# baggepinnen/LPVSpectral.jl

Measured on AMD Instinct MI355X. Metric: signals/sec, ls_sparse_spectral_lpv group lasso N=2^20 Nf=512 Nv=8 (2000 ADMM iters; iters/sec in admm_iters_per_sec), higher is better.
Workload: dtype f64

## Files before the change

lpvspectral.jl_amd/csrc/api.hip:

```cpp
#include <cmath>
#include <cstdarg>
#include <cstdio>
#include <cstdlib>
#include <cstring>
#include <ctime>
#include <map>
#include <mutex>
#include <array>
#include <thread>
#include <string>
#include <vector>

#include "lpvs_internal.h"

namespace lpvs {

static thread_local char g_err[512] = "";

void set_error(const char *fmt, ...) {
    va_list ap;
    va_start(ap, fmt);
    vsnprintf(g_err, sizeof(g_err), fmt, ap);
    va_end(ap);
}
// ... 582 lines not shown
    if (lpvs_device_count() == 0) { set_error("no HIP device visible (the gfx950 path has no CPU fallback)"); return LPVS_EDEVICE; }
    hipStream_t s = nullptr;
    const int64_t nreg = z ? 2 * Nf - 1 : 2 * Nf;
    DevArg dt, df; DevOut dA;
    LPVS_TRY(dt.set(t, N, s)); LPVS_TRY(df.set(f, Nf, s)); LPVS_TRY(dA.set(A_out, N * nreg));
    LPVS_TRY(launch_fourier_regressor_colmajor(dt.p, N, df.p, Nf, (int)z, dA.p, s));
    return dA.finish(s);
}

int32_t lpvs_basis_activation_f64(const double *V, int64_t N, int64_t Nv, int32_t normalize, int32_t coulomb, double *K_out) {
    if (lpvs_device_count() == 0) { set_error("no HIP device visible (the gfx950 path has no CPU fallback)"); return LPVS_EDEVICE; }
    if (N <= 0 || Nv <= 0) { set_error("N and Nv must be positive"); return LPVS_EARGUMENT; }
    hipStream_t s = nullptr;
    const int64_t nb = coulomb ? 2 * Nv : Nv;
    DevArg dV; LPVS_TRY(dV.set(V, N, s));
    double lo, hi, am, gamma; std::vector<double> vc;
    LPVS_TRY(device_minmax(dV.p, N, &lo, &hi, &am, s));
    basis_centers(lo, hi, am, Nv, coulomb, vc, &gamma);
    DevBuf dvc, Kt; LPVS_TRY(dvc.alloc(sizeof(double) * vc.size()));
    LPVS_TRY(copy_to_device(dvc.p, vc.data(), sizeof(double) * vc.size(), s));
    LPVS_TRY(Kt.alloc(sizeof(double) * (size_t)N * (size_t)nb));
    LPVS_TRY(launch_basis_table(dV.p, N, dvc.as<double>(), nb, gamma, normalize, coulomb, Kt.as<double>(), nb, s));
    std::vector<double> hk((size_t)N * nb), ho((size_t)N * nb);
    LPVS_TRY(copy_from_device(hk.data(), Kt.p, sizeof(double) * hk.size(), s));
    for (int64_t n = 0; n < N; ++n) for (int64_t j = 0; j < nb; ++j) ho[n + j * N] = hk[n * nb + j];
    if (is_device_ptr(K_out)) { LPVS_HIP(hipMemcpy(K_out, ho.data(), sizeof(double) * ho.size(), hipMemcpyHostToDevice)); }
    else memcpy(K_out, ho.data(), sizeof(double) * ho.size());
    return LPVS_OK;
}

static int32_t build_lpv_tables(const double *dX, const double *dV, int64_t N, int64_t Npad, const double *dw, int64_t Nf,
                                int64_t Nv, int normalize, int coulomb, DevBuf &T, DevBuf &K, int64_t *ldk_out, hipStream_t s,
                                const double *ranges = nullptr) {
    const int64_t nb = coulomb ? 2 * Nv : Nv, ldk = nb + 1;
    double lo, hi, am, gamma; std::vector<double> vc;
    if (ranges) { lo = ranges[0]; hi = ranges[1]; am = ranges[2]; }
    else LPVS_TRY(device_minmax(dV, N, &lo, &hi, &am, s));
    basis_centers(lo, hi, am, Nv, coulomb, vc, &gamma);
    DevBuf dvc; LPVS_TRY(dvc.alloc(sizeof(double) * vc.size()));
    LPVS_TRY(copy_to_device(dvc.p, vc.data(), sizeof(double) * vc.size(), s));
    LPVS_TRY(T.alloc(sizeof(double2) * (size_t)Npad * (size_t)Nf));
    LPVS_TRY(K.alloc(sizeof(double) * (size_t)Npad * (size_t)ldk));
    if (Npad > N) {
        LPVS_HIP(hipMemsetAsync(T.as<double2>() + N * Nf, 0, sizeof(double2) * (size_t)(Npad - N) * (size_t)Nf, s));
        LPVS_HIP(hipMemsetAsync(K.as<double>() + N * ldk, 0, sizeof(double) * (size_t)(Npad - N) * (size_t)ldk, s));
    }
    LPVS_TRY(launch_trig_table(dX, N, dw, Nf, T.as<double2>(), s));
    LPVS_TRY(launch_basis_table(dV, N, dvc.as<double>(), nb, gamma, normalize, coulomb, K.as<double>(), ldk, s));
    LPVS_HIP(hipStreamSynchronize(s));
    *ldk_out = ldk;
    return LPVS_OK;
}

int32_t lpvs_lpv_regressor_f64(const double *X, const double *V, int64_t N, const double *w, int64_t Nf, int64_t Nv,
                               int32_t normalize, int32_t coulomb, int32_t permuted, double *Phi_out) {
    if (lpvs_device_count() == 0) { set_error("no HIP device visible (the gfx950 path has no CPU fallback)"); return LPVS_EDEVICE; }
    if (N <= 0 || Nf <= 0 || Nv <= 0) { set_error("N, Nf and Nv must be positive"); return LPVS_EARGUMENT; }
    hipStream_t s = nullptr;
    const int64_t nb = coulomb ? 2 * Nv : Nv;
    DevArg dX, dV, dw; DevOut dP;
    LPVS_TRY(dX.set(X, N, s)); LPVS_TRY(dV.set(V, N, s)); LPVS_TRY(dw.set(w, Nf, s));
    LPVS_TRY(dP.set(Phi_out, N * 2 * Nf * nb));
    DevBuf T, K; int64_t ldk;
    LPVS_TRY(build_lpv_tables(dX.p, dV.p, N, N, dw.p, Nf, Nv, normalize, coulomb, T, K, &ldk, s));
    LPVS_TRY(launch_lpv_regressor_colmajor(T.as<double2>(), K.as<double>(), ldk, N, Nf, nb, permuted, dP.p, s));
    return dP.finish(s);
}

struct ApSlots {
    bool ok = false;
    double emax = 0;
    int64_t nf8 = 0, s8 = 0, nsl = 0;
    bool merged = false;
    int64_t s0 = 0;
    double delta = 0;
    std::vector<double> eps, om_hi, om_lo, omr_hi, omr_lo;
    ApStep step{};
};
static thread_local bool g_f32_admission = false;

static ApSlots make_ap_slots(const std::vector<double> &hw, double xam) {
    ApSlots sl;
    const int64_t Nf = (int64_t)hw.size();
    const long double a0 = hw[0], D = Nf > 1 ? ((long double)hw[Nf - 1] - (long double)hw[0]) / (long double)(Nf - 1) : 0.0L;
    sl.eps.resize((size_t)Nf);
    for (int64_t f = 0; f < Nf; ++f) {
        sl.eps[f] = (double)((long double)hw[f] - (a0 + (long double)f * D));
        sl.emax = std::fmax(sl.emax, std::fabs(sl.eps[f]));
    }
    double wam = 0;
    for (double v : hw) wam = std::fmax(wam, std::fabs(v));
    sl.ok = std::isfinite(sl.emax) && std::isfinite(xam) && sl.emax * xam <= 1e-7;
    if (!sl.ok && g_f32_admission && std::isfinite(sl.emax) && std::isfinite(xam) && sl.emax <= 0x1p-23 * wam) {
        sl.ok = true;
        if (sl.emax * xam > 3e-3) for (auto &e : sl.eps) e = 0.0;
    }
    if (!sl.ok) return sl;
    sl.nf8 = round_up(Nf, 8); sl.s8 = round_up(2 * Nf - 1, 8); sl.nsl = sl.nf8 + sl.s8;
    auto split = [](long double v, double &hi, double &lo) { hi = (double)v; lo = (double)(v - (long double)hi); };
    sl.omr_hi.resize((size_t)sl.nf8); sl.omr_lo.resize((size_t)sl.nf8);
    sl.s0 = sl.nf8;
    bool merged = false;
    if (Nf > 1 && D != 0.0L) {
        const long double j0r = 2.0L * a0 / D;
        const long long j0 = llroundl(j0r);
        const long double delta = 2.0L * a0 - (long double)j0 * D;
        if (j0 >= 0 && j0 < Nf && std::fabs((double)delta) * xam <= 1e-7) {
            merged = true; sl.merged = true;
            sl.s0 = j0; sl.delta = (double)delta;
            sl.nsl = round_up(j0 + 2 * Nf - 1, 8);
            sl.s8 = sl.nsl;
        }
    }
    sl.om_hi.resize((size_t)sl.nsl); sl.om_lo.resize((size_t)sl.nsl);
    if (merged) {
        for (int64_t j = 0; j < sl.nsl; ++j) split((long double)j * D, sl.om_hi[j], sl.om_lo[j]);
    } else {
        for (int64_t m = 0; m < sl.nf8; ++m) split((long double)m * D, sl.om_hi[m], sl.om_lo[m]);
        for (int64_t q = 0; q < sl.s8; ++q) split(2.0L * a0 + (long double)q * D, sl.om_hi[sl.nf8 + q], sl.om_lo[sl.nf8 + q]);
    }
    for (int64_t f = 0; f < sl.nf8; ++f) split(a0 + (long double)f * D, sl.omr_hi[f], sl.omr_lo[f]);
    for (int b = 0; b < 8; ++b) split((long double)b * D, sl.step.hi[b], sl.step.lo[b]);
    return sl;
}
struct ApSlotsDev {
    DevBuf hi, lo, rhi, rlo, eps;
    int32_t upload(const ApSlots &sl, hipStream_t s) {
        LPVS_TRY(hi.alloc(sizeof(double) * (size_t)sl.nsl)); LPVS_TRY(lo.alloc(sizeof(double) * (size_t)sl.nsl));
        LPVS_TRY(rhi.alloc(sizeof(double) * (size_t)sl.nf8)); LPVS_TRY(rlo.alloc(sizeof(double) * (size_t)sl.nf8));
        LPVS_TRY(eps.alloc(sizeof(double) * sl.eps.size()));
        LPVS_TRY(copy_to_device(hi.p, sl.om_hi.data(), sizeof(double) * (size_t)sl.nsl, s));
        LPVS_TRY(copy_to_device(lo.p, sl.om_lo.data(), sizeof(double) * (size_t)sl.nsl, s));
        LPVS_TRY(copy_to_device(rhi.p, sl.omr_hi.data(), sizeof(double) * (size_t)sl.nf8, s));
        LPVS_TRY(copy_to_device(rlo.p, sl.omr_lo.data(), sizeof(double) * (size_t)sl.nf8, s));
        LPVS_TRY(copy_to_device(eps.p, sl.eps.data(), sizeof(double) * sl.eps.size(), s));
        return LPVS_OK;
    }
};

static int32_t create_lpv_impl(const double *y, int64_t ns, const double *X, const double *V, int64_t N, const double *w, int64_t Nf,
                               int64_t Nv, int32_t normalize, int32_t coulomb, int32_t device, lpvs_problem **out,
                               const double *ranges = nullptr) {
    if (N <= 0 || Nf <= 0 || Nv <= 0 || ns <= 0) { set_error("N, Nf, Nv and the number of signals must be positive"); return LPVS_EARGUMENT; }
    lpvs_problem *h = nullptr;
    LPVS_TRY(problem_begin(device, out, &h));
    struct Guard { lpvs_problem *h; ~Guard() { delete h; } } guard{h};
    hipStream_t s = h->stream;
    const int64_t nb = coulomb ? 2 * Nv : Nv;
    h->kind = 1; h->N = N; h->Nf = Nf; h->nb = nb; h->n = 2 * Nf * nb; h->np = round_up(h->n, 128); h->ns = ns;
    DevArg dy, dX, dV, dw;
    LPVS_TRY(dy.set(y, N * ns, s)); LPVS_TRY(dX.set(X, N, s)); LPVS_TRY(dV.set(V, N, s)); LPVS_TRY(dw.set(w, Nf, s));
    LPVS_TRY(h->G.alloc(sizeof(double) * (size_t)h->np * (size_t)h->np));
    LPVS_TRY(h->b.alloc(sizeof(double) * (size_t)h->np * (size_t)ns));
    LPVS_HIP(hipMemsetAsync(h->G.p, 0, h->G.bytes, s));
    LPVS_HIP(hipMemsetAsync(h->b.p, 0, h->b.bytes, s));
    LPVS_TRY(alloc_state(h));

    const int form_opt = option_in_effect(LPVS_OPT_GRAM_FORM, h->opt[LPVS_OPT_GRAM_FORM]);
    const std::string form = form_opt == LPVS_GRAM_AP ? "ap" : form_opt == LPVS_GRAM_KRS ? "krs" : form_opt == LPVS_GRAM_KR ? "kr" : "auto";
    bool use_ap = false;
    ApSlots sl;
    double xam = 0;
    if (form == "auto" || form == "ap") {
        std::vector<double> hw;
        LPVS_TRY(fetch_host(hw, w, Nf));
        double xlo, xhi;
        if (ranges) xam = ranges[3];
        else LPVS_TRY(device_minmax(dX.p, N, &xlo, &xhi, &xam, s));
        sl = make_ap_slots(hw, xam);
        use_ap = sl.ok;
        if (form == "ap" && !use_ap) { set_error("LPVS_GRAM_FORM=ap but w is not an arithmetic progression (max|eps|*max|x| = %.3g)", sl.emax * xam); return LPVS_EARGUMENT; }
    }
    if (use_ap) {
        const int64_t nf8 = sl.nf8, nsl = sl.nsl, P = nb * (nb + 1) / 2;
        const ApStep &step = sl.step;
        double lo, hi, am, gamma; std::vector<double> vc;
        DevBuf K, KK, dvc, part, tab, tabb, nwork, epsr;
        ApSlotsDev sd;
        DrainOnExit drain(s);
        LPVS_HIP(hipEventRecord(h->ev[0].a, s));
        if (ranges) { lo = ranges[0]; hi = ranges[1]; am = ranges[2]; }
        else LPVS_TRY(device_minmax(dV.p, N, &lo, &hi, &am, s));
        basis_centers(lo, hi, am, Nv, coulomb, vc, &gamma);
        const int64_t ldk = nb + 1;
        LPVS_TRY(dvc.alloc(sizeof(double) * vc.size()));
        LPVS_TRY(copy_to_device(dvc.p, vc.data(), sizeof(double) * vc.size(), s));
        LPVS_TRY(K.alloc(sizeof(double) * (size_t)N * (size_t)ldk));
        LPVS_TRY(KK.alloc(sizeof(double) * (size_t)N * (size_t)P));
        LPVS_TRY(launch_basis_table(dV.p, N, dvc.as<double>(), nb, gamma, normalize, coulomb, K.as<double>(), ldk, s));
        LPVS_TRY(launch_pair_table(K.as<double>(), ldk, nb, N, KK.as<double>(), s));
        LPVS_TRY(sd.upload(sl, s));
        LPVS_HIP(hipEventRecord(h->ev[0].b, s));
        LPVS_TRY(part.alloc(std::max(nudft_partial_bytes(N, nsl, P), nudft_partial_bytes(N, nf8, nb))));
        LPVS_TRY(tab.alloc(sizeof(double) * (size_t)nsl * (size_t)P * 4));
        LPVS_TRY(tabb.alloc(sizeof(double) * (size_t)nf8 * (size_t)nb * 4));
        LPVS_HIP(hipEventRecord(h->ev[1].a, s));
        const bool nufft_on = option_in_effect(LPVS_OPT_SLOT_SUMS, h->opt[LPVS_OPT_SLOT_SUMS]) != LPVS_SLOTS_DIRECT;
        bool nufft = nufft_on && sl.merged && nufft_applicable(N, nsl, P);
        const int nfg = nufft_grid_size(nsl);
        const double xam_ = xam;
        if (nufft) {
            LPVS_TRY(nwork.alloc(nufft_work_bytes(N, nsl, P)));
            const int32_t rc = launch_nufft_tab(dX.p, nullptr, N, xam_, KK.as<double>(), P, (int)P, step.hi[1], step.lo[1], 0, (int)nsl, nfg, false, nwork.p,
                                                tab.as<double>(), s);
            if (rc == kNufftNonFinite) nufft = false;
            else if (rc != LPVS_OK) return rc;
        }
        if (nufft) {
            h->gram_form = 5;
        } else {
            h->gram_form = 4;
            LPVS_TRY(launch_nudft(dX.p, nullptr, N, KK.as<double>(), P, (int)P, sd.hi.as<double>(), sd.lo.as<double>(), (int)nsl, step, part.as<double>(), tab.as<double>(), s));
        }
        LPVS_TRY(launch_ap_assemble(tab.as<double>(), sd.eps.as<double>(), Nf, sl.s0, sl.delta, nb, h->n, h->G.as<double>(), h->np, s));
        LPVS_HIP(hipEventRecord(h->ev[1].b, s));
        LPVS_HIP(hipEventRecord(h->ev[2].a, s));
        const bool nufft_rhs = nufft && sl.s0 % 2 == 0 && (int)(sl.s0 / 2 + nf8) <= (int)nsl;
        if (nufft_rhs) {
            std::vector<double> er(sl.eps.size());
            for (size_t f = 0; f < er.size(); ++f) er[f] = sl.eps[f] + 0.5 * sl.delta;
            LPVS_TRY(epsr.alloc(sizeof(double) * er.size()));
            LPVS_TRY(copy_to_device(epsr.p, er.data(), sizeof(double) * er.size(), s));
            LPVS_HIP(hipStreamSynchronize(s));
        }
        for (int64_t q = 0; q < ns; ++q) {
            bool by_nufft = nufft_rhs;
            if (by_nufft) {
                const int32_t rc = launch_nufft_tab(dX.p, dy.p + q * N, N, xam_, K.as<double>(), ldk, (int)nb, step.hi[1], step.lo[1], (int)(sl.s0 / 2), (int)nf8, nfg,
                                                    true, nwork.p, tabb.as<double>(), s);
                if (rc == kNufftNonFinite) by_nufft = false;
                else if (rc != LPVS_OK) return rc;
            }
            if (!by_nufft)
                LPVS_TRY(launch_nudft(dX.p, dy.p + q * N, N, K.as<double>(), ldk, (int)nb, sd.rhi.as<double>(), sd.rlo.as<double>(), (int)nf8, step, part.as<double>(), tabb.as<double>(), s));
            LPVS_TRY(launch_ap_rhs(tabb.as<double>(), by_nufft ? epsr.as<double>() : sd.eps.as<double>(), Nf, nb, h->b.as<double>() + q * h->np, s));
        }
        LPVS_HIP(hipEventRecord(h->ev[2].b, s));
        LPVS_HIP(hipStreamSynchronize(s));
        h->t_basis = h->ev[0].ms(); h->t_gram = h->ev[1].ms(); h->t_reduce = h->ev[2].ms();
        h->gram_launches = 8.0 * (double)N * (double)nsl * (double)P;
        h->gram_flops = (double)N * (double)h->n * (double)(h->n + 1);
        guard.h = nullptr;
        *out = h;
        return LPVS_OK;
    }

    const bool krs = form != "kr" && gram_krs_fits(nb);
    const GramPlan pl = krs ? make_gram_plan_pairs(Nf, nb, N) : make_gram_plan(h->n, N);
    const int64_t Npad = pl.ksplit * pl.rows_per_chunk;

    DevBuf T, K, KK, G3, slab, scr; int64_t ldk;
    DrainOnExit drain(s);
    LPVS_HIP(hipEventRecord(h->ev[0].a, s));
    LPVS_TRY(build_lpv_tables(dX.p, dV.p, N, Npad, dw.p, Nf, Nv, normalize, coulomb, T, K, &ldk, s, ranges));
    if (krs) {
        LPVS_TRY(KK.alloc(sizeof(double) * (size_t)Npad * (size_t)pl.pairs));
        LPVS_TRY(launch_pair_table(K.as<double>(), ldk, nb, Npad, KK.as<double>(), s));
    }
    LPVS_HIP(hipEventRecord(h->ev[0].b, s));
    LPVS_TRY(slab.alloc(pl.slab_bytes));
    LPVS_TRY(scr.alloc(rhs_scratch_bytes(N, h->n)));
    if (krs) LPVS_TRY(G3.alloc(sizeof(double) * (size_t)pl.np2 * (size_t)(pl.np2 * pl.pairs)));
    struct Side { hipStream_t s = nullptr; hipEvent_t ready = nullptr, done = nullptr;
                  ~Side() { if (s) { (void)hipStreamSynchronize(s); (void)hipStreamDestroy(s); } if (ready) (void)hipEventDestroy(ready); if (done) (void)hipEventDestroy(done); } } side;
    LPVS_HIP(hipStreamCreateWithFlags(&side.s, hipStreamNonBlocking));
    LPVS_HIP(hipEventCreateWithFlags(&side.ready, hipEventDisableTiming));
    LPVS_HIP(hipEventCreateWithFlags(&side.done, hipEventDisableTiming));
    LPVS_HIP(hipEventRecord(side.ready, s));
    LPVS_HIP(hipStreamWaitEvent(side.s, side.ready, 0));
    LPVS_HIP(hipEventRecord(h->ev[1].a, s));
    if (krs) LPVS_TRY(launch_gram_krs(pl, T.as<double2>(), Nf, KK.as<double>(), nb, slab.as<double>(), s));
    else LPVS_TRY(launch_gram_kr(pl, T.as<double2>(), Nf, K.as<double>(), ldk, nb, slab.as<double>(), s));
    LPVS_HIP(hipEventRecord(h->ev[1].b, s));
    for (int64_t q = 0; q < ns; ++q)
        LPVS_TRY(launch_rhs_kr(T.as<double2>(), Nf, K.as<double>(), ldk, nb, dy.p + q * N, N, h->b.as<double>() + q * h->np, scr.as<double>(), scr.bytes, side.s));
    LPVS_HIP(hipEventRecord(side.done, side.s));
    LPVS_HIP(hipEventRecord(h->ev[2].a, s));
    if (krs) LPVS_TRY(launch_gram_reduce_krs(pl, slab.as<double>(), nb, G3.as<double>(), h->G.as<double>(), h->np, s));
    else LPVS_TRY(launch_gram_reduce(pl, slab.as<double>(), h->G.as<double>(), h->np, s));
    LPVS_HIP(hipStreamWaitEvent(s, side.done, 0));
    LPVS_HIP(hipEventRecord(h->ev[2].b, s));
    LPVS_HIP(hipStreamSynchronize(s));
    h->t_basis = h->ev[0].ms(); h->t_gram = h->ev[1].ms(); h->t_reduce = h->ev[2].ms();
    h->gram_launches = (double)pl.tiles * 128.0 * 256.0 * 2.0 * (double)(pl.ksplit * pl.rows_per_chunk); h->gram_flops = (double)N * (double)h->n * (double)(h->n + 1);
    h->gram_form = krs ? 2 : 1;
    guard.h = nullptr;
    *out = h;
    return LPVS_OK;
}

int32_t lpvs_problem_create_lpv_f64(const double *y, const double *X, const double *V, int64_t N, const double *w, int64_t Nf,
                                    int64_t Nv, int32_t normalize, int32_t coulomb, int32_t device, lpvs_problem **out) {
    return create_lpv_impl(y, 1, X, V, N, w, Nf, Nv, normalize, coulomb, device, out);
}

int32_t lpvs_problem_create_lpv_multi_f64(const double *Y, int64_t ns, const double *X, const double *V, int64_t N, const double *w,
                                          int64_t Nf, int64_t Nv, int32_t normalize, int32_t coulomb, int32_t device,
                                          lpvs_problem **out) {
    return create_lpv_impl(Y, ns, X, V, N, w, Nf, Nv, normalize, coulomb, device, out);
}

int32_t lpvs_lpv_ranges_f64(const double *X, const double *V, int64_t N, double *out4) {
    if (!X || !V || !out4 || N <= 0) { set_error("NULL argument or N <= 0"); return LPVS_EARGUMENT; }
    if (lpvs_device_count() == 0) { set_error("no HIP device visible (the gfx950 path has no CPU fallback)"); return LPVS_EDEVICE; }
    hipStream_t s = nullptr;
    DevArg dX, dV;
    LPVS_TRY(dX.set(X, N, s)); LPVS_TRY(dV.set(V, N, s));
    double xlo, xhi;
    LPVS_TRY(device_minmax(dV.p, N, &out4[0], &out4[1], &out4[2], s));
    LPVS_TRY(device_minmax(dX.p, N, &xlo, &xhi, &out4[3], s));
    return LPVS_OK;
}

int32_t lpvs_problem_create_lpv_rows_f64(const double *Y, int64_t ns, const double *X, const double *V, int64_t N_local, const double *w,
                                         int64_t Nf, int64_t Nv, int32_t normalize, int32_t coulomb, const double *ranges4,
                                         int32_t device, lpvs_problem **out) {
    if (!ranges4) { set_error("ranges4 is NULL"); return LPVS_EARGUMENT; }
    if (!(ranges4[0] <= ranges4[1]) || !(ranges4[2] >= 0) || !(ranges4[3] >= 0)) { set_error("ranges4 = {min V, max V, max|V|, max|X|} is inconsistent"); return LPVS_EARGUMENT; }
    return create_lpv_impl(Y, ns, X, V, N_local, w, Nf, Nv, normalize, coulomb, device, out, ranges4);
}

int32_t lpvs_problem_device_gram_f64(lpvs_problem *h, double **G_dev, double **b_dev, int64_t *np) {
    if (!h) { set_error("NULL handle"); return LPVS_EARGUMENT; }
    if (G_dev) *G_dev = h->G.as<double>();
    if (b_dev) *b_dev = h->b.as<double>();
    if (np) *np = h->np;
    return LPVS_OK;
}

int32_t lpvs_problem_gram_modified(lpvs_problem *h) {
    if (!h) { set_error("NULL handle"); return LPVS_EARGUMENT; }
    h->M_valid = false; h->Mp_valid = false; h->inited = false;
    h->drop_graph();
    return LPVS_OK;
}

int32_t lpvs_problem_create_fourier_f64(const double *y, const double *t, int64_t N, const double *f, int64_t Nf, const double *W,
                                        int32_t device, lpvs_problem **out) {
    if (N <= 0 || Nf <= 0) { set_error("N and Nf must be positive"); return LPVS_EARGUMENT; }
    int64_t zf = 0;
    LPVS_TRY(lpvs_check_freq_f64(f, Nf, &zf));
    lpvs_problem *h = nullptr;
    LPVS_TRY(problem_begin(device, out, &h));
    struct Guard { lpvs_problem *h; ~Guard() { delete h; } } guard{h};
    hipStream_t s = h->stream;
    h->kind = 0; h->N = N; h->Nf = Nf; h->zerofreq = zf; h->n = zf ? 2 * Nf - 1 : 2 * Nf;
    DevArg dt, df;
    LPVS_TRY(dt.set(t, N, s)); LPVS_TRY(df.set(f, Nf, s));
    const int form_opt = option_in_effect(LPVS_OPT_GRAM_FORM, h->opt[LPVS_OPT_GRAM_FORM]);
    const std::string form = form_opt == LPVS_GRAM_AP ? "ap" : form_opt == LPVS_GRAM_KRS ? "krs" : form_opt == LPVS_GRAM_KR ? "kr" : "auto";
    if (form == "auto" || form == "ap") {
        std::vector<double> hw;
        LPVS_TRY(fetch_host(hw, f, Nf));
        for (auto &v : hw) v = 6.283185307179586 * v;
        double tlo, thi, tam;
        LPVS_TRY(device_minmax(dt.p, N, &tlo, &thi, &tam, s));
        const ApSlots sl = make_ap_slots(hw, tam);
        if (form == "ap" && !sl.ok) { set_error("LPVS_GRAM_FORM=ap but 2*pi*f is not an arithmetic progression (max|eps|*max|t| = %.3g)", sl.emax * tam); return LPVS_EARGUMENT; }
        if (sl.ok) {
            h->np = round_up(h->n, 128);
            DevArg dy, dW;
            LPVS_TRY(dy.set(y, N, s));
            if (W) LPVS_TRY(dW.set(W, N, s));
            LPVS_TRY(h->G.alloc(sizeof(double) * (size_t)h->np * (size_t)h->np));
            LPVS_TRY(h->b.alloc(sizeof(double) * (size_t)h->np));
            LPVS_HIP(hipMemsetAsync(h->G.p, 0, h->G.bytes, s));
            LPVS_HIP(hipMemsetAsync(h->b.p, 0, h->b.bytes, s));
            LPVS_TRY(alloc_state(h));
            ApSlotsDev sd; DevBuf part, tab, tabb;
            DrainOnExit drain(s);
            LPVS_HIP(hipEventRecord(h->ev[0].a, s));
            LPVS_TRY(sd.upload(sl, s));
            LPVS_HIP(hipEventRecord(h->ev[0].b, s));
            LPVS_TRY(part.alloc(std::max(nudft_partial_bytes(N, sl.nsl, 1), nudft_partial_bytes(N, sl.nf8, 1))));
            LPVS_TRY(tab.alloc(sizeof(double) * (size_t)sl.nsl * 4));
            LPVS_TRY(tabb.alloc(sizeof(double) * (size_t)sl.nf8 * 4));
            const double *Wd = W ? dW.p : nullptr;
            LPVS_HIP(hipEventRecord(h->ev[1].a, s));
            LPVS_TRY(launch_nudft(dt.p, nullptr, N, Wd, 1, 1, sd.hi.as<double>(), sd.lo.as<double>(), (int)sl.nsl, sl.step, part.as<double>(), tab.as<double>(), s));
            LPVS_TRY(launch_ap_assemble_fourier(tab.as<double>(), sd.eps.as<double>(), Nf, sl.s0, sl.delta, (int)zf, h->n, h->G.as<double>(), h->np, 1, 0, 0, s));
            LPVS_HIP(hipEventRecord(h->ev[1].b, s));
            LPVS_HIP(hipEventRecord(h->ev[2].a, s));
            LPVS_TRY(launch_nudft(dt.p, dy.p, N, Wd, 1, 1, sd.rhi.as<double>(), sd.rlo.as<double>(), (int)sl.nf8, sl.step, part.as<double>(), tabb.as<double>(), s));
            LPVS_TRY(launch_ap_rhs_fourier(tabb.as<double>(), sd.eps.as<double>(), Nf, (int)zf, h->b.as<double>(), 1, 0, 0, s));
            LPVS_HIP(hipEventRecord(h->ev[2].b, s));
            LPVS_HIP(hipStreamSynchronize(s));
            h->t_basis = h->ev[0].ms(); h->t_gram = h->ev[1].ms(); h->t_reduce = h->ev[2].ms();
            h->gram_launches = 8.0 * (double)N * (double)sl.nsl;
            h->gram_flops = (double)N * (double)h->n * (double)(h->n + 1);
            h->gram_form = 4;
            guard.h = nullptr;
            *out = h;
            return LPVS_OK;
        }
    }
    LPVS_TRY(create_panel_problem(h, y, W, N, [&](double *P, int64_t ld) {
        return launch_fourier_panel(dt.p, N, df.p, Nf, (int)zf, P, ld, s);
    }));
    guard.h = nullptr;
// ... 1444 lines not shown
```

lpvspectral.jl_amd/csrc/nudft.hip:

```cpp
#include "lpvs_internal.h"

#include <cstdlib>

namespace lpvs {

namespace {

constexpr int RB = 16;

template <int QPT, int S>
__global__ void __launch_bounds__(256)
nudft_accumulate_kernel(const double *__restrict__ x, const double *__restrict__ y, int64_t N, const double *__restrict__ Wt,
                        int64_t ldw, int nq, const double *__restrict__ om_hi, const double *__restrict__ om_lo, int nslots,
                        const ApStep step, double *__restrict__ out, const int64_t *__restrict__ seg, int64_t rows_per_chunk) {
    constexpr int SLOTS = 64 * S, NA = 8 * S;
    constexpr int WSTR = (QPT + 1) & ~1;
    constexpr int NEF = NA + 8;
    __shared__ __attribute__((aligned(16))) double wrow[2][RB][4 * WSTR];
    __shared__ __attribute__((aligned(16))) double ef[2][RB][NEF][2];
    __shared__ double xs[2][RB], ys[2][RB];
    const int t = threadIdx.x;
    const int sl = t & 63;
    const int g = __builtin_amdgcn_readfirstlane(t >> 6);
    const int slot0 = blockIdx.x * SLOTS;
// ... 41 lines not shown
            }
            ef[buf][pr][pk][0] = c; ef[buf][pr][pk][1] = sn;
        }
        for (int e = t; e < RB * 4 * QPT; e += 256) {
            const int pr = e / (4 * QPT), q = e - pr * (4 * QPT);
            const int64_t r = rb + pr;
            const double wv = (r < r1 && q < nqb) ? (Wt ? Wt[(r - wbase) * ldw + qbase + q] : 1.0) : 0.0;
            wrow[buf][pr][(q / QPT) * WSTR + q % QPT] = wv;
        }
        __syncthreads();
        if (nvalid > 0) {
#pragma unroll
            for (int rr = 0; rr < RB; ++rr) {
                const double yv = ys[buf][rr], xv = xs[buf][rr];
                double tv[S][4];
#pragma unroll
                for (int u = 0; u < S; ++u) {
                    const int ls = sl + 64 * u;
                    const double2 e2 = *reinterpret_cast<const double2 *>(&ef[buf][rr][ls >> 3][0]);
                    const double2 f2 = *reinterpret_cast<const double2 *>(&ef[buf][rr][NA + (ls & 7)][0]);
                    const double c = fma(e2.x, f2.x, -(e2.y * f2.y)) * yv, sn = fma(e2.y, f2.x, e2.x * f2.y) * yv;
                    tv[u][0] = c; tv[u][1] = sn; tv[u][2] = xv * c; tv[u][3] = xv * sn;
                }
                double wq[WSTR];
#pragma unroll
                for (int q = 0; q < WSTR; q += 2) {
                    const double2 w2 = *reinterpret_cast<const double2 *>(&wrow[buf][rr][g * WSTR + q]);
                    wq[q] = w2.x; wq[q + 1] = w2.y;
                }
#pragma unroll
                for (int q = 0; q < QPT; ++q)
#pragma unroll
                    for (int u = 0; u < S; ++u) {
                        acc[u][q][0] = fma(wq[q], tv[u][0], acc[u][q][0]);
                        acc[u][q][1] = fma(wq[q], tv[u][1], acc[u][q][1]);
                        acc[u][q][2] = fma(wq[q], tv[u][2], acc[u][q][2]);
                        acc[u][q][3] = fma(wq[q], tv[u][3], acc[u][q][3]);
                    }
            }
        }
    }
    if (nvalid > 0) {
#pragma unroll
        for (int u = 0; u < S; ++u) {
            const int slot = slot0 + sl + 64 * u;
            if (slot >= nslots) continue;
            double *o = out + (((int64_t)blockIdx.y * nslots + slot) * nq + qbase + q0) * 4;
#pragma unroll
            for (int q = 0; q < QPT; ++q)
                if (q < nvalid) {
#pragma unroll
                    for (int v = 0; v < 4; ++v) o[q * 4 + v] = acc[u][q][v];
                }
        }
    }
}


template <int S>
__global__ void __launch_bounds__(256)
nudft_single_kernel(const double *__restrict__ x, const double *__restrict__ y, int64_t N, const double *__restrict__ Wt, int64_t ldw,
                    const double *__restrict__ om_hi, const double *__restrict__ om_lo, int nslots, const ApStep step,
                    double *__restrict__ out, const int64_t *__restrict__ seg, int64_t rows_per_chunk) {
    constexpr int NA = 8 * S, NEF = NA + 8;
    __shared__ __attribute__((aligned(16))) double ef[2][RB][NEF][2];
    __shared__ double xs[2][RB], ws[2][RB];
    __shared__ __attribute__((aligned(16))) double comb[3][64 * S][4];
    const int t = threadIdx.x, sl = t & 63;
    const int g = __builtin_amdgcn_readfirstlane(t >> 6);
    const int slot0 = blockIdx.x * 64 * S;
    int64_t r0 = (int64_t)blockIdx.y * rows_per_chunk;
    int64_t r1 = r0 + rows_per_chunk < N ? r0 + rows_per_chunk : N;
    int64_t wbase = 0;
    if (seg != nullptr) { r0 = seg[3 * blockIdx.y]; r1 = seg[3 * blockIdx.y + 1]; wbase = seg[3 * blockIdx.y + 2]; }
    double acc[S][4];
#pragma unroll
    for (int u = 0; u < S; ++u)
#pragma unroll
        for (int v = 0; v < 4; ++v) acc[u][v] = 0.0;
    int buf = 0;
    for (int64_t rb = r0; rb < r1; rb += RB, buf ^= 1) {
        for (int e = t; e < RB * NEF; e += 256) {
            const int pr = e / NEF, pk = e - pr * NEF;
            double wh, wl;
            if (pk < NA) {
                const int as = slot0 + 8 * pk;
                const bool ok = as < nslots;
                wh = ok ? om_hi[as] : 0.0; wl = ok ? om_lo[as] : 0.0;
            } else {
                wh = step.hi[pk - NA]; wl = step.lo[pk - NA];
            }
            const int64_t r = rb + pr;
            double c = 1.0, sn = 0.0;
            if (r < r1) {
                const double xv = x[r];
                const double p = wh * xv;
                const double d = fma(wh, xv, -p) + wl * xv;
                sincos(p, &sn, &c);
                const double c2 = fma(-d, sn, c), s2 = fma(d, c, sn);
                c = c2; sn = s2;
                if (pk == 0) { xs[buf][pr] = xv; ws[buf][pr] = (Wt ? Wt[(r - wbase) * ldw] : 1.0) * (y ? y[r] : 1.0); }
            } else if (pk == 0) {
                xs[buf][pr] = 0.0; ws[buf][pr] = 0.0;
            }
            ef[buf][pr][pk][0] = c; ef[buf][pr][pk][1] = sn;
        }
        __syncthreads();
#pragma unroll
        for (int i = 0; i < RB / 4; ++i) {
            const int rr = g + 4 * i;
            const double wv = ws[buf][rr], xv = xs[buf][rr];
#pragma unroll
            for (int u = 0; u < S; ++u) {
                const int ls = sl + 64 * u;
                const double2 e2 = *reinterpret_cast<const double2 *>(&ef[buf][rr][ls >> 3][0]);
                const double2 f2 = *reinterpret_cast<const double2 *>(&ef[buf][rr][NA + (ls & 7)][0]);
                const double c = fma(e2.x, f2.x, -(e2.y * f2.y)) * wv, sn = fma(e2.y, f2.x, e2.x * f2.y) * wv;
                acc[u][0] += c; acc[u][1] += sn;
                acc[u][2] = fma(xv, c, acc[u][2]); acc[u][3] = fma(xv, sn, acc[u][3]);
            }
        }
    }
    __syncthreads();
    if (g > 0) {
#pragma unroll
        for (int u = 0; u < S; ++u) {
            double4 o; o.x = acc[u][0]; o.y = acc[u][1]; o.z = acc[u][2]; o.w = acc[u][3];
            *reinterpret_cast<double4 *>(&comb[g - 1][sl + 64 * u][0]) = o;
        }
    }
    __syncthreads();
    if (g == 0) {
#pragma unroll
        for (int u = 0; u < S; ++u) {
            const int slot = slot0 + sl + 64 * u;
            if (slot >= nslots) continue;
            double *o = out + ((int64_t)blockIdx.y * nslots + slot) * 4;
#pragma unroll
            for (int v = 0; v < 4; ++v) o[v] = ((acc[u][v] + comb[0][sl + 64 * u][v]) + comb[1][sl + 64 * u][v]) + comb[2][sl + 64 * u][v];
        }
    }
}

__global__ void __launch_bounds__(256)
nudft_reduce_kernel(const double *__restrict__ part_all, int nchunks, int64_t count, double *__restrict__ out_all) {
    const int64_t i = (int64_t)blockIdx.x * 256 + threadIdx.x;
    if (i >= count) return;
    const double *part = part_all + (int64_t)blockIdx.y * nchunks * count;
    double s = 0;
    for (int c = 0; c < nchunks; ++c) s += part[(int64_t)c * count + i];
    out_all[(int64_t)blockIdx.y * count + i] = s;
}

__global__ void __launch_bounds__(256)
ap_assemble_fourier_kernel(const double *__restrict__ tab_all, const double *__restrict__ eps, int Nf, int s0, double delta, int zf, double scale,
                           int64_t n, double *__restrict__ G_all, int64_t ldg, int64_t tab_stride, int64_t g_stride) {
    const int64_t ga = blockIdx.y;
    const int64_t gb = (int64_t)blockIdx.x * 256 + threadIdx.x;
    if (gb > ga || ga >= n) return;
    const double *tab = tab_all + (int64_t)blockIdx.z * tab_stride;
    double *G = G_all + (int64_t)blockIdx.z * g_stride;
    const int ca = ga >= Nf, cb = gb >= Nf;
    const int ka = ca ? (int)ga - Nf + zf : (int)ga, kb = cb ? (int)gb - Nf + zf : (int)gb;
    const int hi = ka >= kb ? ka : kb, lo = ka >= kb ? kb : ka;
    const double dm = eps[hi] - eps[lo], dp = (eps[ka] + eps[kb]) + delta;
    const double *tm = tab + (int64_t)(hi - lo) * 4;
    const double *tp = tab + (int64_t)(s0 + ka + kb) * 4;
    const double cm = fma(-dm, tm[3], tm[0]);
    double sm = fma(dm, tm[2], tm[1]);
    if (ka < kb) sm = -sm;
    const double cp = fma(-dp, tp[3], tp[0]), sp = fma(dp, tp[2], tp[1]);
    double v;
    if (!ca && !cb) v = 0.5 * (cm + cp);
    else if (ca && cb) v = 0.5 * (cm - cp);
    else if (!ca && cb) v = -0.5 * (sp - sm);
    else v = -0.5 * (sp + sm);
    v *= scale;
    G[ga * ldg + gb] = v;
    G[gb * ldg + ga] = v;
}

__global__ void __launch_bounds__(256)
ap_rhs_fourier_kernel(const double *__restrict__ tab_all, const double *__restrict__ eps, int Nf, int zf, double dd,
                      double *__restrict__ b_all, int64_t tab_stride, int64_t b_stride) {
    const int k = blockIdx.x * 256 + threadIdx.x;
    if (k >= Nf) return;
    const double *t = tab_all + (int64_t)blockIdx.y * tab_stride + (int64_t)k * 4;
    double *b = b_all + (int64_t)blockIdx.y * b_stride;
    const double e = eps[k];
    b[k] = dd * fma(-e, t[3], t[0]);
    if (k >= zf) b[Nf + k - zf] = -dd * fma(e, t[2], t[1]);
}

__global__ void __launch_bounds__(256)
ap_assemble_kernel(const double *__restrict__ tab, const double *__restrict__ eps, int Nf, int s0, double delta, int nb, int P, int64_t n,
                   double *__restrict__ G, int64_t ldg) {
    const int64_t ga = blockIdx.y;
    const int64_t gb = (int64_t)blockIdx.x * 256 + threadIdx.x;
    if (gb > ga || ga >= n) return;
    const int g2 = 2 * nb;
    const int fa = (int)(ga / g2), ra = (int)(ga - (int64_t)fa * g2), ca = ra >= nb, ja0 = ra - ca * nb;
    const int fb = (int)(gb / g2), rbm = (int)(gb - (int64_t)fb * g2), cb = rbm >= nb, jb0 = rbm - cb * nb;
    int ja = ja0, jb = jb0;
    if (ja > jb) { const int t = ja; ja = jb; jb = t; }
    const int q = ja * nb - ja * (ja - 1) / 2 + (jb - ja);
    const int m = fa - fb, s = fa + fb;
    const double dm = eps[fa] - eps[fb], dp = (eps[fa] + eps[fb]) + delta;
    const double *tm = tab + ((int64_t)m * P + q) * 4;
    const double *tp = tab + ((int64_t)(s0 + s) * P + q) * 4;
    const double cm = fma(-dm, tm[3], tm[0]), sm = fma(dm, tm[2], tm[1]);
    const double cp = fma(-dp, tp[3], tp[0]), sp = fma(dp, tp[2], tp[1]);
    double v;
    if (!ca && !cb) v = 0.5 * (cm + cp);
    else if (ca && cb) v = 0.5 * (cm - cp);
    else if (!ca && cb) v = -0.5 * (sp - sm);
    else v = -0.5 * (sp + sm);
    G[ga * ldg + gb] = v;
    G[gb * ldg + ga] = v;
}

__global__ void __launch_bounds__(256)
ap_rhs_kernel(const double *__restrict__ tab, const double *__restrict__ eps, int Nf, int nb, double *__restrict__ b) {
    const int i = blockIdx.x * 256 + threadIdx.x;
    if (i >= Nf * nb) return;
    const int f = i / nb, j = i - f * nb;
    const double *t = tab + ((int64_t)f * nb + j) * 4;
    const double e = eps[f];
    b[(int64_t)f * 2 * nb + j] = fma(-e, t[3], t[0]);
    b[(int64_t)f * 2 * nb + nb + j] = -fma(e, t[2], t[1]);
}

template <int QPT, int S>
void launch_accumulate(unsigned nchunks, hipStream_t s, const double *x, const double *y, int64_t N, const double *Wt, int64_t ldw, int nq,
                       const double *om_hi, const double *om_lo, int nslots, const ApStep &step, double *partial, const int64_t *seg,
                       int64_t rpc) {
    dim3 grid((unsigned)ceil_div(nslots, 64 * S), nchunks, (unsigned)ceil_div(nq, 4 * QPT));
    hipLaunchKernelGGL((nudft_accumulate_kernel<QPT, S>), grid, dim3(256), 0, s, x, y, N, Wt, ldw, nq, om_hi, om_lo, nslots, step, partial, seg, rpc);
}

}

int64_t nudft_rows_per_chunk(int64_t N, int64_t nslots) {
    const int64_t groups = ceil_div(nslots, 128);
    int64_t rpc = 8192;
    while (rpc > 64 && groups * ceil_div(N, rpc) < 2048) rpc >>= 1;
    return rpc;
}
size_t nudft_chunks(int64_t N, int64_t nslots) { return (size_t)ceil_div(N, nudft_rows_per_chunk(N, nslots)); }
size_t nudft_partial_bytes(int64_t N, int64_t nslots, int64_t nq) {
    return sizeof(double) * nudft_chunks(N, nslots) * (size_t)nslots * (size_t)nq * 4;
}

static int32_t nudft_impl(const double *x, const double *y, int64_t N, const double *Wt, int64_t ldw, int nq, const double *om_hi,
                          const double *om_lo, int nslots, const ApStep &step, double *partial, double *tab, const int64_t *seg,
                          unsigned nseg, unsigned nbatch, hipStream_t s) {
    if (nslots % 8 != 0) { set_error("nudft: slot count %d is not a multiple of 8", nslots); return LPVS_ESTATE; }
    const unsigned nchunks = seg ? nseg : (unsigned)nudft_chunks(N, nslots);
    const int64_t rpc = seg ? 0 : nudft_rows_per_chunk(N, nslots);
    if (nq == 1) {
        dim3 grid((unsigned)ceil_div(nslots, 128), nchunks, 1);
        hipLaunchKernelGGL(nudft_single_kernel<2>, grid, dim3(256), 0, s, x, y, N, Wt, ldw, om_hi, om_lo, nslots, step, partial, seg, rpc);
    } else if (nq <= 8) launch_accumulate<2, 2>(nchunks, s, x, y, N, Wt, ldw, nq, om_hi, om_lo, nslots, step, partial, seg, rpc);
    else if (nq <= 16) launch_accumulate<4, 2>(nchunks, s, x, y, N, Wt, ldw, nq, om_hi, om_lo, nslots, step, partial, seg, rpc);
    else launch_accumulate<9, 2>(nchunks, s, x, y, N, Wt, ldw, nq, om_hi, om_lo, nslots, step, partial, seg, rpc);
    LPVS_HIP(hipGetLastError());
    const int64_t count = (int64_t)nslots * nq * 4;
    hipLaunchKernelGGL(nudft_reduce_kernel, dim3((unsigned)ceil_div(count, 256), nbatch), dim3(256), 0, s, partial, (int)(nchunks / nbatch), count, tab);
    LPVS_HIP(hipGetLastError());
    return LPVS_OK;
}

int32_t launch_nudft(const double *x, const double *y, int64_t N, const double *Wt, int64_t ldw, int nq, const double *om_hi,
                     const double *om_lo, int nslots, const ApStep &step, double *partial, double *tab, hipStream_t s) {
    return nudft_impl(x, y, N, Wt, ldw, nq, om_hi, om_lo, nslots, step, partial, tab, nullptr, 0, 1, s);
}

int32_t launch_nudft_windows(const double *x, const double *y, const double *Wt, const double *om_hi, const double *om_lo, int nslots,
                             const ApStep &step, const int64_t *seg_dev, int nwin, int segs_per_window, double *partial, double *tab,
                             hipStream_t s) {
    return nudft_impl(x, y, 0, Wt, 1, 1, om_hi, om_lo, nslots, step, partial, tab, seg_dev, (unsigned)(nwin * segs_per_window), (unsigned)nwin, s);
}

int32_t launch_ap_assemble_fourier(const double *tab, const double *eps, int64_t Nf, int64_t s0, double delta, int zf, int64_t n, double *G,
                                   int64_t ldg, int nbatch, int64_t tab_stride, int64_t g_stride, hipStream_t s) {
    dim3 grid((unsigned)ceil_div(n, 256), (unsigned)n, (unsigned)nbatch);
    hipLaunchKernelGGL(ap_assemble_fourier_kernel, grid, dim3(256), 0, s, tab, eps, (int)Nf, (int)s0, delta, zf, 1.0 / (double)(2 * Nf), n, G, ldg,
                       tab_stride, g_stride);
    LPVS_HIP(hipGetLastError());
    return LPVS_OK;
}

int32_t launch_ap_rhs_fourier(const double *tab, const double *eps, int64_t Nf, int zf, double *b, int nbatch, int64_t tab_stride,
                              int64_t b_stride, hipStream_t s) {
    hipLaunchKernelGGL(ap_rhs_fourier_kernel, dim3((unsigned)ceil_div(Nf, 256), (unsigned)nbatch), dim3(256), 0, s, tab, eps, (int)Nf, zf,
                       1.0 / sqrt((double)(2 * Nf)), b, tab_stride, b_stride);
    LPVS_HIP(hipGetLastError());
    return LPVS_OK;
}

int32_t launch_ap_assemble(const double *tab, const double *eps, int64_t Nf, int64_t s0, double delta, int64_t nb, int64_t n, double *G,
                           int64_t ldg, hipStream_t s) {
    const int P = (int)(nb * (nb + 1) / 2);
    dim3 grid((unsigned)ceil_div(n, 256), (unsigned)n);
    hipLaunchKernelGGL(ap_assemble_kernel, grid, dim3(256), 0, s, tab, eps, (int)Nf, (int)s0, delta, (int)nb, P, n, G, ldg);
    LPVS_HIP(hipGetLastError());
    return LPVS_OK;
}

int32_t launch_ap_rhs(const double *tab, const double *eps, int64_t Nf, int64_t nb, double *b, hipStream_t s) {
    hipLaunchKernelGGL(ap_rhs_kernel, dim3((unsigned)ceil_div(Nf * nb, 256)), dim3(256), 0, s, tab, eps, (int)Nf, (int)nb, b);
    LPVS_HIP(hipGetLastError());
    return LPVS_OK;
}

}
```

Measured before the change: 15.31.

## Tile Gram assembly over lower-triangular blocks with shared-memory transpose; trim memset

The AP Gram assembly kernels now run one 64x64 lower-triangular tile per block and write the mirrored upper half through a shared-memory transpose, so both stores are coalesced. Before, each thread wrote G[gb*ldg+ga] as a strided scatter, and half the launched threads exited early. The full G memset is also removed from the AP path; only the padding rows and columns are zeroed there, and the full memset stays on the non-AP path. This is setup cost only. The timed metric is ADMM iterations, so the change may make little difference to the measured throughput.

Result: no change. 15.31 (-0.0%).

```diff
diff --git a/lpvspectral.jl_amd/csrc/api.hip b/lpvspectral.jl_amd/csrc/api.hip
--- a/lpvspectral.jl_amd/csrc/api.hip
+++ b/lpvspectral.jl_amd/csrc/api.hip
@@ -758,7 +758,6 @@
     LPVS_TRY(dy.set(y, N * ns, s)); LPVS_TRY(dX.set(X, N, s)); LPVS_TRY(dV.set(V, N, s)); LPVS_TRY(dw.set(w, Nf, s));
     LPVS_TRY(h->G.alloc(sizeof(double) * (size_t)h->np * (size_t)h->np));
     LPVS_TRY(h->b.alloc(sizeof(double) * (size_t)h->np * (size_t)ns));
-    LPVS_HIP(hipMemsetAsync(h->G.p, 0, h->G.bytes, s));
     LPVS_HIP(hipMemsetAsync(h->b.p, 0, h->b.bytes, s));
     LPVS_TRY(alloc_state(h));
 
@@ -778,6 +777,11 @@
         if (form == "ap" && !use_ap) { set_error("LPVS_GRAM_FORM=ap but w is not an arithmetic progression (max|eps|*max|x| = %.3g)", sl.emax * xam); return LPVS_EARGUMENT; }
     }
     if (use_ap) {
+        if (h->np > h->n) {
+            double *Gp = h->G.as<double>();
+            LPVS_HIP(hipMemsetAsync(Gp + h->n * h->np, 0, sizeof(double) * (size_t)(h->np - h->n) * (size_t)h->np, s));
+            LPVS_HIP(hipMemset2DAsync(Gp + h->n, sizeof(double) * (size_t)h->np, 0, sizeof(double) * (size_t)(h->np - h->n), (size_t)h->n, s));
+        }
         const int64_t nf8 = sl.nf8, nsl = sl.nsl, P = nb * (nb + 1) / 2;
         const ApStep &step = sl.step;
         double lo, hi, am, gamma; std::vector<double> vc;
@@ -851,6 +855,7 @@
         return LPVS_OK;
     }
 
+    LPVS_HIP(hipMemsetAsync(h->G.p, 0, h->G.bytes, s));
     const bool krs = form != "kr" && gram_krs_fits(nb);
     const GramPlan pl = krs ? make_gram_plan_pairs(Nf, nb, N) : make_gram_plan(h->n, N);
     const int64_t Npad = pl.ksplit * pl.rows_per_chunk;
diff --git a/lpvspectral.jl_amd/csrc/nudft.hip b/lpvspectral.jl_amd/csrc/nudft.hip
--- a/lpvspectral.jl_amd/csrc/nudft.hip
+++ b/lpvspectral.jl_amd/csrc/nudft.hip
@@ -217,32 +217,63 @@
     out_all[(int64_t)blockIdx.y * count + i] = s;
 }
 
+constexpr int AT = 64;
+
+template <class Entry>
+static __device__ __forceinline__ void ap_assemble_tile(const Entry &entry, int64_t n, double *__restrict__ G, int64_t ldg) {
+    __shared__ double tile[AT][AT + 1];
+    int ti = (int)((sqrt(8.0 * (double)blockIdx.x + 1.0) - 1.0) * 0.5);
+    while ((int64_t)ti * (ti + 1) / 2 > (int64_t)blockIdx.x) --ti;
+    while ((int64_t)(ti + 1) * (ti + 2) / 2 <= (int64_t)blockIdx.x) ++ti;
+    const int tj = (int)((int64_t)blockIdx.x - (int64_t)ti * (ti + 1) / 2);
+    const int c = threadIdx.x & (AT - 1), r0 = threadIdx.x >> 6;
+    const int64_t a0 = (int64_t)ti * AT, b0 = (int64_t)tj * AT;
+    const bool diag = ti == tj;
+#pragma unroll 4
+    for (int r = r0; r < AT; r += 4) {
+        const int64_t ga = a0 + r, gb = b0 + c;
+        if (ga < n && gb < n && gb <= ga) {
+            const double v = entry(ga, gb);
+            tile[r][c] = v;
+            if (diag) tile[c][r] = v;
+            else G[ga * ldg + gb] = v;
+        }
+    }
+    __syncthreads();
+    if (diag) {
+#pragma unroll 4
+        for (int r = r0; r < AT; r += 4)
+            if (a0 + r < n && a0 + c < n) G[(a0 + r) * ldg + a0 + c] = tile[r][c];
+    } else {
+#pragma unroll 4
+        for (int r = r0; r < AT; r += 4)
+            if (b0 + r < n && a0 + c < n) G[(b0 + r) * ldg + a0 + c] = tile[c][r];
+    }
+}
+static unsigned ap_assemble_tiles(int64_t n) { const int64_t T = ceil_div(n, AT); return (unsigned)(T * (T + 1) / 2); }
+
 __global__ void __launch_bounds__(256)
 ap_assemble_fourier_kernel(const double *__restrict__ tab_all, const double *__restrict__ eps, int Nf, int s0, double delta, int zf, double scale,
                            int64_t n, double *__restrict__ G_all, int64_t ldg, int64_t tab_stride, int64_t g_stride) {
-    const int64_t ga = blockIdx.y;
-    const int64_t gb = (int64_t)blockIdx.x * 256 + threadIdx.x;
-    if (gb > ga || ga >= n) return;
-    const double *tab = tab_all + (int64_t)blockIdx.z * tab_stride;
-    double *G = G_all + (int64_t)blockIdx.z * g_stride;
-    const int ca = ga >= Nf, cb = gb >= Nf;
-    const int ka = ca ? (int)ga - Nf + zf : (int)ga, kb = cb ? (int)gb - Nf + zf : (int)gb;
-    const int hi = ka >= kb ? ka : kb, lo = ka >= kb ? kb : ka;
-    const double dm = eps[hi] - eps[lo], dp = (eps[ka] + eps[kb]) + delta;
-    const double *tm = tab + (int64_t)(hi - lo) * 4;
-    const double *tp = tab + (int64_t)(s0 + ka + kb) * 4;
-    const double cm = fma(-dm, tm[3], tm[0]);
-    double sm = fma(dm, tm[2], tm[1]);
-    if (ka < kb) sm = -sm;
-    const double cp = fma(-dp, tp[3], tp[0]), sp = fma(dp, tp[2], tp[1]);
-    double v;
-    if (!ca && !cb) v = 0.5 * (cm + cp);
-    else if (ca && cb) v = 0.5 * (cm - cp);
-    else if (!ca && cb) v = -0.5 * (sp - sm);
-    else v = -0.5 * (sp + sm);
-    v *= scale;
-    G[ga * ldg + gb] = v;
-    G[gb * ldg + ga] = v;
+    const double *tab = tab_all + (int64_t)blockIdx.y * tab_stride;
+    ap_assemble_tile([&](int64_t ga, int64_t gb) {
+        const int ca = ga >= Nf, cb = gb >= Nf;
+        const int ka = ca ? (int)ga - Nf + zf : (int)ga, kb = cb ? (int)gb - Nf + zf : (int)gb;
+        const int hi = ka >= kb ? ka : kb, lo = ka >= kb ? kb : ka;
+        const double dm = eps[hi] - eps[lo], dp = (eps[ka] + eps[kb]) + delta;
+        const double *tm = tab + (int64_t)(hi - lo) * 4;
+        const double *tp = tab + (int64_t)(s0 + ka + kb) * 4;
+        const double cm = fma(-dm, tm[3], tm[0]);
+        double sm = fma(dm, tm[2], tm[1]);
+        if (ka < kb) sm = -sm;
+        const double cp = fma(-dp, tp[3], tp[0]), sp = fma(dp, tp[2], tp[1]);
+        double v;
+        if (!ca && !cb) v = 0.5 * (cm + cp);
+        else if (ca && cb) v = 0.5 * (cm - cp);
+        else if (!ca && cb) v = -0.5 * (sp - sm);
+        else v = -0.5 * (sp + sm);
+        return v * scale;
+    }, n, G_all + (int64_t)blockIdx.y * g_stride, ldg);
 }
 
 __global__ void __launch_bounds__(256)
@@ -260,28 +291,26 @@
 __global__ void __launch_bounds__(256)
 ap_assemble_kernel(const double *__restrict__ tab, const double *__restrict__ eps, int Nf, int s0, double delta, int nb, int P, int64_t n,
                    double *__restrict__ G, int64_t ldg) {
-    const int64_t ga = blockIdx.y;
-    const int64_t gb = (int64_t)blockIdx.x * 256 + threadIdx.x;
-    if (gb > ga || ga >= n) return;
-    const int g2 = 2 * nb;
-    const int fa = (int)(ga / g2), ra = (int)(ga - (int64_t)fa * g2), ca = ra >= nb, ja0 = ra - ca * nb;
-    const int fb = (int)(gb / g2), rbm = (int)(gb - (int64_t)fb * g2), cb = rbm >= nb, jb0 = rbm - cb * nb;
-    int ja = ja0, jb = jb0;
-    if (ja > jb) { const int t = ja; ja = jb; jb = t; }
-    const int q = ja * nb - ja * (ja - 1) / 2 + (jb - ja);
-    const int m = fa - fb, s = fa + fb;
-    const double dm = eps[fa] - eps[fb], dp = (eps[fa] + eps[fb]) + delta;
-    const double *tm = tab + ((int64_t)m * P + q) * 4;
-    const double *tp = tab + ((int64_t)(s0 + s) * P + q) * 4;
-    const double cm = fma(-dm, tm[3], tm[0]), sm = fma(dm, tm[2], tm[1]);
-    const double cp = fma(-dp, tp[3], tp[0]), sp = fma(dp, tp[2], tp[1]);
-    double v;
-    if (!ca && !cb) v = 0.5 * (cm + cp);
-    else if (ca && cb) v = 0.5 * (cm - cp);
-    else if (!ca && cb) v = -0.5 * (sp - sm);
-    else v = -0.5 * (sp + sm);
-    G[ga * ldg + gb] = v;
-    G[gb * ldg + ga] = v;
+    ap_assemble_tile([&](int64_t ga, int64_t gb) {
+        const int g2 = 2 * nb;
+        const int fa = (int)(ga / g2), ra = (int)(ga - (int64_t)fa * g2), ca = ra >= nb, ja0 = ra - ca * nb;
+        const int fb = (int)(gb / g2), rbm = (int)(gb - (int64_t)fb * g2), cb = rbm >= nb, jb0 = rbm - cb * nb;
+        int ja = ja0, jb = jb0;
+        if (ja > jb) { const int t = ja; ja = jb; jb = t; }
+        const int q = ja * nb - ja * (ja - 1) / 2 + (jb - ja);
+        const int m = fa - fb, s = fa + fb;
+        const double dm = eps[fa] - eps[fb], dp = (eps[fa] + eps[fb]) + delta;
+        const double *tm = tab + ((int64_t)m * P + q) * 4;
+        const double *tp = tab + ((int64_t)(s0 + s) * P + q) * 4;
+        const double cm = fma(-dm, tm[3], tm[0]), sm = fma(dm, tm[2], tm[1]);
+        const double cp = fma(-dp, tp[3], tp[0]), sp = fma(dp, tp[2], tp[1]);
+        double v;
+        if (!ca && !cb) v = 0.5 * (cm + cp);
+        else if (ca && cb) v = 0.5 * (cm - cp);
+        else if (!ca && cb) v = -0.5 * (sp - sm);
+        else v = -0.5 * (sp + sm);
+        return v;
+    }, n, G, ldg);
 }
 
 __global__ void __launch_bounds__(256)
@@ -348,7 +377,7 @@
 
 int32_t launch_ap_assemble_fourier(const double *tab, const double *eps, int64_t Nf, int64_t s0, double delta, int zf, int64_t n, double *G,
                                    int64_t ldg, int nbatch, int64_t tab_stride, int64_t g_stride, hipStream_t s) {
-    dim3 grid((unsigned)ceil_div(n, 256), (unsigned)n, (unsigned)nbatch);
+    dim3 grid(ap_assemble_tiles(n), (unsigned)nbatch);
     hipLaunchKernelGGL(ap_assemble_fourier_kernel, grid, dim3(256), 0, s, tab, eps, (int)Nf, (int)s0, delta, zf, 1.0 / (double)(2 * Nf), n, G, ldg,
                        tab_stride, g_stride);
     LPVS_HIP(hipGetLastError());
@@ -366,7 +395,7 @@
 int32_t launch_ap_assemble(const double *tab, const double *eps, int64_t Nf, int64_t s0, double delta, int64_t nb, int64_t n, double *G,
                            int64_t ldg, hipStream_t s) {
     const int P = (int)(nb * (nb + 1) / 2);
-    dim3 grid((unsigned)ceil_div(n, 256), (unsigned)n);
+    dim3 grid(ap_assemble_tiles(n));
     hipLaunchKernelGGL(ap_assemble_kernel, grid, dim3(256), 0, s, tab, eps, (int)Nf, (int)s0, delta, (int)nb, P, n, G, ldg);
     LPVS_HIP(hipGetLastError());
     return LPVS_OK;
```
